# NVlabs/motion-policy-networks

Measured on AMD Instinct MI355X. Metric: env-steps/sec (FK+SDF+PointNet++), higher is better.
Workload: dtype f32

## Files before the change

### motion-policy-networks_amd/csrc/sa3_chain.hip

```cpp
#include "common.h"

#include <type_traits>

typedef float f32x16 __attribute__((ext_vector_type(16)));
typedef unsigned int u32x4 __attribute__((ext_vector_type(4)));

namespace sa3 {
constexpr int ROWS = 128, PR = 64, WV = 4;

template <int K1, int C1, int C2, int C3>
struct Cfg {
  static_assert(K1 % 8 == 0 && K1 % 16 == 0, "input rows are whole 16-float slabs");
  static_assert(C1 == 128 * WV && C2 == 128 * WV && C3 == 256 * WV, "a wave owns 128 channels (256 of the last layer)");
  static constexpr int KG1 = K1 / 8, KG2 = C1 / 8, KG3 = C2 / 8;
  static constexpr int64_t W1_OFF = 0, W2_OFF = (int64_t)C1 * K1, W3_OFF = W2_OFF + (int64_t)C2 * C1;
  static constexpr int64_t B1_OFF = W3_OFF + (int64_t)C3 * C2, B2_OFF = B1_OFF + C1, B3_OFF = B2_OFF + C2;
  static constexpr int64_t TOTAL = B3_OFF + C3;
  static constexpr int KMAX = K1 > C1 ? (K1 > C2 ? K1 : C2) : (C1 > C2 ? C1 : C2);
  static constexpr int LD = KMAX + 4;
  static constexpr int LDS_BYTES = PR * LD * 4;
};
}

template <class C>
__global__ void __launch_bounds__(256)
    sa3_pack_kernel(const float *__restrict__ w1, int k1_real, const float *__restrict__ b1, const float *__restrict__ w2,
                    const float *__restrict__ b2, const float *__restrict__ w3, const float *__restrict__ b3, int K1, int C1,
                    int C2, int C3, float *__restrict__ pack) {
  const int64_t e = (int64_t)blockIdx.x * 256 + threadIdx.x;
  if (e >= C::TOTAL) return;
  float v;
  if (e >= C::B1_OFF) {
    const int64_t i = e - C::B1_OFF;
    v = i < C1 ? b1[i] : (i < C1 + C2 ? b2[i - C1] : b3[i - C1 - C2]);
  } else {
    const float *w;
    int kin, kreal, KG;
    int64_t r = e;
    if (r >= C::W3_OFF) { r -= C::W3_OFF; w = w3; kin = C2; kreal = C2; KG = C::KG3; }
    else if (r >= C::W2_OFF) { r -= C::W2_OFF; w = w2; kin = C1; kreal = C1; KG = C::KG2; }
    else { w = w1; kin = K1; kreal = k1_real; KG = C::KG1; }
    const int i = (int)(r & 3), lane = (int)((r >> 2) & 63), ot = (int)((r >> 8) & 3);
    const int64_t ug = r >> 10;
    const int g = (int)(ug % KG), unit = (int)(ug / KG);
    const int out = unit * 128 + ot * 32 + (lane & 31), in = 8 * g + 4 * (lane >> 5) + i;
    (void)kin;
    v = in < kreal ? w[(size_t)out * kreal + in] : 0.0f;
  }
  pack[e] = v;
}

__device__ __forceinline__ f32x16 sa3_mfma(float a, float b, f32x16 c) { return __builtin_amdgcn_mfma_f32_32x32x2f32(a, b, c, 0, 0, 0); }
__device__ __forceinline__ float4 sa3_bload16(__amdgpu_buffer_rsrc_t rsrc, int voff, int soff) {
  const u32x4 r = __builtin_amdgcn_raw_buffer_load_b128(rsrc, voff, soff, 0);
  return make_float4(__uint_as_float(r.x), __uint_as_float(r.y), __uint_as_float(r.z), __uint_as_float(r.w));
}
template <int I, int E, class F>
__device__ __forceinline__ void static_for(F &&f) {
  if constexpr (I < E) {
    f(std::integral_constant<int, I>{});
    static_for<I + 1, E>(f);
  }
}
__device__ __forceinline__ float sa3_comp(const float4 &q, int i) { return i == 0 ? q.x : (i == 1 ? q.y : (i == 2 ? q.z : q.w)); }

template <int K1, int C1, int C2, int C3, bool PROBE = false>
__global__ void __launch_bounds__(64 * sa3::WV) __attribute__((amdgpu_waves_per_eu(1, 1)))
    sa3_chain_kernel(const float *__restrict__ x, int ldx, const float *__restrict__ pack, float *__restrict__ out, int ldo,
                     long long *__restrict__ probe = nullptr) {
  using C = sa3::Cfg<K1, C1, C2, C3>;
  using namespace sa3;
  extern __shared__ __attribute__((aligned(16))) float H[];
  constexpr int LD = C::LD;
  const int tid = threadIdx.x, lane = tid & 63;
  const int wave = __builtin_amdgcn_readfirstlane(tid >> 6);
  const int half = lane >> 5, col = lane & 31;
  const int64_t env = blockIdx.x;
  const __amdgpu_buffer_rsrc_t rsrc =
      __builtin_amdgcn_make_buffer_rsrc(const_cast<float *>(pack), 0, (int)(C::TOTAL * 4), 0x00020000);
  const int voff = lane * 16;
  const float *hrow0 = H + col * LD + 4 * half;
  float pool[2][4];
#pragma unroll
  for (int hf = 0; hf < 2; ++hf)
#pragma unroll
    for (int ot = 0; ot < 4; ++ot) pool[hf][ot] = -__builtin_inff();

  auto run = [&](auto KGt, auto FLIPt, int wbase, f32x16 (&acc)[4][2]) __attribute__((always_inline)) {
    constexpr int KG = decltype(KGt)::value;
    constexpr bool FLIP = decltype(FLIPt)::value;
    constexpr int NS = 4;
    float4 wr[NS][4], br[NS][2];
    auto fetch = [&](int st, int g) __attribute__((always_inline)) {
      const int soff = wbase + g * 4096;
#pragma unroll
      for (int ot = 0; ot < 4; ++ot) wr[st][ot] = sa3_bload16(rsrc, voff + ot * 1024, soff);
      br[st][0] = *reinterpret_cast<const float4 *>(hrow0 + 8 * g);
      br[st][1] = *reinterpret_cast<const float4 *>(hrow0 + 32 * LD + 8 * g);
    };
    auto compute = [&](int st) __attribute__((always_inline)) {
#pragma unroll
      for (int i = 0; i < 4; ++i)
#pragma unroll
        for (int ot = 0; ot < 4; ++ot)
#pragma unroll
          for (int rt = 0; rt < 2; ++rt) {
            const float w = sa3_comp(wr[st][ot], i), a = sa3_comp(br[st][rt], i);
            acc[ot][rt] = FLIP ? sa3_mfma(w, a, acc[ot][rt]) : sa3_mfma(a, w, acc[ot][rt]);
          }
    };
#pragma unroll
    for (int st = 0; st < NS - 1; ++st) fetch(st, st);
    auto issue_order = [&]() __attribute__((always_inline)) {
#pragma unroll
      for (int k = 0; k < 4; ++k) {
        __builtin_amdgcn_sched_group_barrier(0x008, 4, 0);
        __builtin_amdgcn_sched_group_barrier(0x020, 1, 0);
      }
#pragma unroll
      for (int k = 0; k < 2; ++k) {
        __builtin_amdgcn_sched_group_barrier(0x008, 4, 0);
        __builtin_amdgcn_sched_group_barrier(0x100, 1, 0);
      }
      __builtin_amdgcn_sched_group_barrier(0x008, 8, 0);
    };
    constexpr int ROUNDS = (KG - NS + 1) / NS;
    for (int r = 0; r < ROUNDS; ++r) {
#pragma unroll
      for (int st = 0; st < NS; ++st) {
        fetch((st + NS - 1) % NS, r * NS + st + NS - 1);
        compute(st);
        issue_order();
      }
    }
    static_for<ROUNDS * NS, KG>([&](auto G) __attribute__((always_inline)) {
      constexpr int g = decltype(G)::value;
      if constexpr (g + NS - 1 < KG) {
        fetch((g + NS - 1) % NS, g + NS - 1);
        compute(g % NS);
        issue_order();
      } else {
        compute(g % NS);
      }
    });
  };
  auto bias_init = [&](int boff_floats, f32x16 (&acc)[4][2]) __attribute__((always_inline)) {
#pragma unroll
    for (int ot = 0; ot < 4; ++ot)
#pragma unroll
      for (int j = 0; j < 4; ++j) {
        const float4 b = sa3_bload16(rsrc, half * 16, (boff_floats + wave * 128 + ot * 32 + 8 * j) * 4);
#pragma unroll
        for (int rt = 0; rt < 2; ++rt) {
          acc[ot][rt][4 * j + 0] = b.x, acc[ot][rt][4 * j + 1] = b.y, acc[ot][rt][4 * j + 2] = b.z, acc[ot][rt][4 * j + 3] = b.w;
        }
      }
  };
  auto write_back = [&](const f32x16 (&acc)[4][2]) __attribute__((always_inline)) {
#pragma unroll
    for (int rt = 0; rt < 2; ++rt)
#pragma unroll
      for (int ot = 0; ot < 4; ++ot)
#pragma unroll
        for (int j = 0; j < 4; ++j) {
          float4 v;
          v.x = fmaxf(acc[ot][rt][4 * j + 0], 0.0f), v.y = fmaxf(acc[ot][rt][4 * j + 1], 0.0f);
          v.z = fmaxf(acc[ot][rt][4 * j + 2], 0.0f), v.w = fmaxf(acc[ot][rt][4 * j + 3], 0.0f);
          *reinterpret_cast<float4 *>(H + (rt * 32 + col) * LD + wave * 128 + ot * 32 + 8 * j + 4 * half) = v;
        }
  };

  int pi = 0;
  auto stamp = [&]() __attribute__((always_inline)) {
    if constexpr (PROBE) {
      if (blockIdx.x == 300 && tid == 0) probe[pi] = (long long)__builtin_amdgcn_s_memtime();
      ++pi;
    }
  };
  stamp();
  for (int pass = 0; pass < ROWS / PR; ++pass) {
    const float *xr = x + (env * ROWS + pass * PR) * (int64_t)ldx;
    constexpr int NX = PR * (K1 / 4) / (64 * WV);
    static_assert(NX * 64 * WV == PR * (K1 / 4), "the input rows split evenly over the threads");
    {
      float4 xb[NX];
#pragma unroll
      for (int j = 0; j < NX; ++j) {
        const int i = tid + j * 64 * WV, r = i / (K1 / 4), c4 = i - r * (K1 / 4);
        xb[j] = *reinterpret_cast<const float4 *>(xr + (int64_t)r * ldx + 4 * c4);
      }
#pragma unroll
      for (int j = 0; j < NX; ++j) {
        const int i = tid + j * 64 * WV, r = i / (K1 / 4), c4 = i - r * (K1 / 4);
        *reinterpret_cast<float4 *>(H + r * LD + 4 * c4) = xb[j];
      }
    }
    __syncthreads();
    stamp();
    f32x16 acc[4][2];
    bias_init((int)C::B1_OFF, acc);
    run(std::integral_constant<int, C::KG1>{}, std::true_type{}, (int)(C::W1_OFF * 4) + wave * C::KG1 * 4096, acc);
    stamp();
    __syncthreads();
    write_back(acc);
    __syncthreads();
    stamp();
    bias_init((int)C::B2_OFF, acc);
    run(std::integral_constant<int, C::KG2>{}, std::true_type{}, (int)(C::W2_OFF * 4) + wave * C::KG2 * 4096, acc);
    stamp();
    __syncthreads();
    write_back(acc);
    __syncthreads();
    stamp();
#pragma unroll
    for (int hf = 0; hf < 2; ++hf) {
#pragma unroll
      for (int ot = 0; ot < 4; ++ot)
#pragma unroll
        for (int rt = 0; rt < 2; ++rt) acc[ot][rt] = f32x16{0, 0, 0, 0, 0, 0, 0, 0, 0, 0, 0, 0, 0, 0, 0, 0};
      run(std::integral_constant<int, C::KG3>{}, std::false_type{}, (int)(C::W3_OFF * 4) + (wave * 2 + hf) * C::KG3 * 4096, acc);
#pragma unroll
      for (int ot = 0; ot < 4; ++ot) {
        float m = fmaxf(acc[ot][0][0], acc[ot][1][0]);
#pragma unroll
        for (int r = 1; r < 16; ++r) m = fmaxf(m, fmaxf(acc[ot][0][r], acc[ot][1][r]));
        pool[hf][ot] = fmaxf(pool[hf][ot], m);
      }
      stamp();
    }
    __syncthreads();
    stamp();
  }
  const float *b3 = pack + C::B3_OFF;
#pragma unroll
  for (int hf = 0; hf < 2; ++hf)
#pragma unroll
    for (int ot = 0; ot < 4; ++ot) {
      const float v = mpx_max_across_halves(pool[hf][ot]);
      const int ch = wave * 256 + hf * 128 + ot * 32 + col;
      if (half == 0) out[env * (int64_t)ldo + ch] = fmaxf(v + b3[ch], 0.0f);
    }
}

#define SA3_DISPATCH(CALL)                                                                              \
  if (K1 == 272 && c1 == 512 && c2 == 512 && c3 == 1024) { CALL(272, 512, 512, 1024); }                 \
  else {                                                                                                \
    mpx_set_error("mpx_sa3: unsupported group-all MLP (K1=%d, %d, %d, %d)", K1, c1, c2, c3);            \
    return 1;                                                                                           \
  }

MPX_EXPORT int64_t mpx_sa3_pack_size(int K1, int c1, int c2, int c3) {
  if (K1 == 272 && c1 == 512 && c2 == 512 && c3 == 1024) return sa3::Cfg<272, 512, 512, 1024>::TOTAL;
  return -1;
}

MPX_EXPORT int mpx_sa3_pack_weights(const float *w1, int k1_real, const float *b1, const float *w2, const float *b2,
                                    const float *w3, const float *b3, int K1, int c1, int c2, int c3, float *pack,
                                    mpx_stream_t stream) {
  MPX_REQUIRE(w1 && b1 && w2 && b2 && w3 && b3 && pack, "mpx_sa3_pack_weights: NULL operand");
  MPX_REQUIRE(k1_real >= 1 && k1_real <= K1, "mpx_sa3_pack_weights: the real input width %d must be in [1, K1 = %d]", k1_real, K1);
#define CALL(a, b, c, d)                                                                                             \
  do {                                                                                                               \
    using C = sa3::Cfg<a, b, c, d>;                                                                                  \
    hipLaunchKernelGGL(sa3_pack_kernel<C>, dim3(cdiv(C::TOTAL, 256)), dim3(256), 0, mpx_s(stream), w1, k1_real, b1, w2, \
                       b2, w3, b3, K1, c1, c2, c3, pack);                                                            \
    MPX_LAUNCH_CHECK("mpx_sa3_pack_weights");                                                                        \
  } while (0)
  SA3_DISPATCH(CALL)
#undef CALL
}

MPX_EXPORT int mpx_sa3_chain_probe(const float *x, int ldx, int B, const float *pack, float *out, int ldo, int64_t *probe,
                                   mpx_stream_t stream) {
  using C = sa3::Cfg<272, 512, 512, 1024>;
  MPX_LDS_LIMIT_ONCE((sa3_chain_kernel<272, 512, 512, 1024, true>), C::LDS_BYTES, "mpx_sa3_chain_probe");
  hipLaunchKernelGGL((sa3_chain_kernel<272, 512, 512, 1024, true>), dim3((unsigned)B), dim3(64 * sa3::WV), C::LDS_BYTES,
                     mpx_s(stream), x, ldx, pack, out, ldo, reinterpret_cast<long long *>(probe));
  MPX_LAUNCH_CHECK("mpx_sa3_chain_probe");
}

MPX_EXPORT int mpx_sa3_chain(const float *x, int ldx, int B, int rows, const float *pack, int K1, int c1, int c2, int c3,
                             float *out, int ldo, mpx_stream_t stream) {
  MPX_REQUIRE(B >= 0 && x && pack && out, "mpx_sa3_chain: bad operand");
  MPX_REQUIRE(rows == sa3::ROWS, "mpx_sa3_chain: the module pools exactly %d rows per environment (got %d)", sa3::ROWS, rows);
  MPX_REQUIRE(ldx >= K1 && ldx % 4 == 0 && ldo >= c3, "mpx_sa3_chain: bad leading dimension");
  MPX_REQUIRE((((uintptr_t)x | (uintptr_t)pack) & 15) == 0, "mpx_sa3_chain: x and pack must be 16-byte aligned");
  if (B == 0) return 0;
#define CALL(a, b, c, d)                                                                                            \
  do {                                                                                                              \
    using C = sa3::Cfg<a, b, c, d>;                                                                                 \
    MPX_LDS_LIMIT_ONCE((sa3_chain_kernel<a, b, c, d>), C::LDS_BYTES, "mpx_sa3_chain");                              \
    hipLaunchKernelGGL((sa3_chain_kernel<a, b, c, d>), dim3((unsigned)B), dim3(64 * sa3::WV), C::LDS_BYTES,        \
                       mpx_s(stream), x, ldx, pack, out, ldo, (long long *)nullptr);                                \
    MPX_LAUNCH_CHECK("mpx_sa3_chain");                                                                              \
  } while (0)
  SA3_DISPATCH(CALL)
#undef CALL
}
```

### motion-policy-networks_amd/csrc/launch_routes.h

```cpp
#pragma once
#include <stdint.h>

static inline int cdiv(int64_t a, int64_t b) { return (int)((a + b - 1) / b); }

#ifndef MPX_FPS4_MIN_B
#define MPX_FPS4_MIN_B 768
#endif
constexpr int FPS_MAX_N = 8192;
constexpr int FPS_MAX_LDS = 256 + 3 * FPS_MAX_N * 4;
constexpr int FPSC_CELLS = 4096;
constexpr int64_t fpsc_lds_bytes(int N, bool nocloud = false) {
  const int64_t cloud = nocloud ? 0 : (int64_t)3 * N * 4, pro = (int64_t)FPSC_CELLS * 4 + (((int64_t)N * 2 + 15) & ~(int64_t)15);
  return 768 + (cloud > pro ? cloud : pro);
}
inline int opt_n_threads_log2(int n) {
  int l = 0;
  while ((2 << l) <= n && (2 << l) <= 512) ++l;
  return l;
}

enum { FPS_PLAIN = 0, FPS_WAVE = 1, FPS_CULL8 = 2, FPS_CULL4 = 3 };
struct FpsRoute {
  int family;
  int pts;
  int threads;
  int lds;
};
inline FpsRoute fps_route(int B, int N, int fast) {
  if (fast && N <= 512) {
    switch ((N + 63) / 64) {
      case 1: return {FPS_WAVE, 1, 64, 0};
      case 2: return {FPS_WAVE, 2, 64, 0};
      case 3: case 4: return {FPS_WAVE, 4, 64, 0};
      default: return {FPS_WAVE, 8, 64, 0};
    }
  }
  if (fast && N > 512) {
    const int waves = (N > 16 * 256 && B >= MPX_FPS4_MIN_B) ? 4 : 8;
    const int lds_c = (int)fpsc_lds_bytes(N, waves == 4);
    const int pts_c = (N + 64 * waves - 1) / (64 * waves);
    if (waves == 4) return {FPS_CULL4, pts_c <= 20 ? 20 : pts_c <= 25 ? 25 : 32, 256, lds_c};
    const int p = pts_c <= 2 ? 2 : pts_c <= 4 ? 4 : pts_c <= 6 ? 6 : pts_c <= 8 ? 8 : pts_c <= 10 ? 10 : pts_c <= 13 ? 13 : 16;
    return {FPS_CULL8, p, 512, lds_c};
  }
  int block = ((N + 63) / 64) * 64;
  if (block > 512) block = 512;
  const int pts = (N + block - 1) / block;
  const int lds = 256 + 3 * N * 4;
  switch (pts) {
    case 1: case 2: case 3: case 4: case 5: case 6: case 7: case 8: return {FPS_PLAIN, pts, block, lds};
    case 9: case 10: return {FPS_PLAIN, 10, block, lds};
    case 11: case 12: case 13: return {FPS_PLAIN, 13, block, lds};
    case 14: case 15: case 16: return {FPS_PLAIN, 16, block, lds};
    default: return {FPS_PLAIN, 0, block, lds};
  }
}

constexpr int COL_PPB = 16;
#ifndef MPX_COL_TC
#define MPX_COL_TC 64
#endif
static_assert(MPX_COL_TC >= 1 && MPX_COL_TC <= 64 && MPX_COL_TC * 64 <= 16 * 256,
              "MPX_COL_TC: FK runs on one thread per waypoint of a chunk and a thread holds at most 16 (waypoint, sphere) pairs");

enum { COL_NONE = 0, COL_GENERAL = 1, COL_WAVE = 2, COL_ENV = 3 };
struct CollisionRoute {
  int form;
  int ppt;
  int block;
  int tc;
  int chunks;
  int last;
};
inline CollisionRoute collision_route(int B, int T, int S, int M1, int M2, bool frames_aligned) {
  if (B == 0 || T == 0 || S == 0) return {COL_NONE, 0, 0, 0, 0, 0};
  if (M1 <= 64 && M2 <= 64 && S <= 64 && frames_aligned) {
    const bool wave = T * S <= 64;
    const int tc = wave ? 64 : MPX_COL_TC;
    const int chunks = cdiv(T, tc), last = (T - (chunks - 1) * tc) * S;
    if (wave) return {COL_WAVE, 1, 64, tc, chunks, last};
    const int sel = ((T < tc ? T : tc) * S + 511) / 512;
    return {COL_ENV, sel >= 1 && sel <= 7 ? 2 * sel : 16, 256, tc, chunks, last};
  }
  const int groups = cdiv((int64_t)B * T, COL_PPB);
  return {COL_GENERAL, 0, 256, 0, groups, (int)((int64_t)B * T - (int64_t)(groups - 1) * COL_PPB) * S};
}

constexpr int LINEAR_BM = 128, LINEAR_BN = 128;
inline bool gemv_fits(int M, int K) { return M <= 8 && (int64_t)(M <= 1 ? 1 : M <= 2 ? 2 : M <= 4 ? 4 : 8) * K * 4 <= 64 * 1024; }
// ... 101 lines not shown
```

### motion-policy-networks_amd/csrc/pointnet.hip

```cpp
#include "common.h"

#include <stdlib.h>
#include <type_traits>

typedef unsigned long long u64;

template <int CTRL>
__device__ __forceinline__ u64 dpp_mov64(u64 v) {
  unsigned lo = (unsigned)v, hi = (unsigned)(v >> 32);
  lo = (unsigned)__builtin_amdgcn_update_dpp(0, (int)lo, CTRL, 0xf, 0xf, true);
  hi = (unsigned)__builtin_amdgcn_update_dpp(0, (int)hi, CTRL, 0xf, 0xf, true);
  return ((u64)hi << 32) | lo;
}
struct U32Pair {
  unsigned lo, hi;
};
__device__ __forceinline__ u64 pack64(unsigned lo, unsigned hi) { return __builtin_bit_cast(u64, U32Pair{lo, hi}); }
__device__ __forceinline__ u64 umax64(u64 a, u64 b) {
  double r;
  asm("v_max_f64 %0, %1, %2" : "=v"(r) : "v"(__builtin_bit_cast(double, a)), "v"(__builtin_bit_cast(double, b)));
  return __builtin_bit_cast(u64, r);
}

__device__ __forceinline__ u64 row_max64(u64 v) {
  v = umax64(v, dpp_mov64<0xB1>(v));
  v = umax64(v, dpp_mov64<0x4E>(v));
  v = umax64(v, dpp_mov64<0x141>(v));
  v = umax64(v, dpp_mov64<0x140>(v));
  return v;
}
__device__ __forceinline__ u64 readlane64(u64 v, int lane) {
  unsigned lo = (unsigned)__builtin_amdgcn_readlane((int)(unsigned)v, lane);
  unsigned hi = (unsigned)__builtin_amdgcn_readlane((int)(unsigned)(v >> 32), lane);
  return ((u64)hi << 32) | lo;
}
__device__ __forceinline__ u64 wave_max64(u64 v) {
  v = row_max64(v);
  u64 a = umax64(readlane64(v, 0), readlane64(v, 16));
  u64 b = umax64(readlane64(v, 32), readlane64(v, 48));
  return umax64(a, b);
}

template <int PTS>
__global__ void __launch_bounds__(1024) __attribute__((amdgpu_waves_per_eu(PTS <= 8 ? 8 : 4, PTS <= 8 ? 8 : 4)))
    fps_kernel(const float *__restrict__ xyz, int N, int stride, int npoint, int log2bs,
               int32_t *__restrict__ idx, float *__restrict__ new_xyz, int new_stride) {
  extern __shared__ __attribute__((aligned(16))) unsigned char smem[];
  u64 *slots = reinterpret_cast<u64 *>(smem);
  float *sx = reinterpret_cast<float *>(smem + 256);
  float *sy = sx + N;
  float *sz = sy + N;

  const int b = blockIdx.x;
  const int tid = threadIdx.x;
  const int nthr = blockDim.x;
  const int lane = tid & 63;
  const int wave = tid >> 6;
  const float *pts = xyz + (size_t)b * N * stride;
  int32_t *out = idx + (size_t)b * npoint;
  float *nxyz = new_xyz ? new_xyz + (size_t)b * npoint * new_stride : nullptr;
  const unsigned bsmask = (1u << log2bs) - 1u;

  float x[PTS], y[PTS], z[PTS];
  u64 key[PTS];
#pragma unroll
  for (int i = 0; i < PTS; ++i) {
    const int k = tid + i * nthr;
    x[i] = y[i] = z[i] = 0.0f;
    key[i] = 0;
    if (k < N) {
      x[i] = pts[(size_t)k * stride + 0];
      y[i] = pts[(size_t)k * stride + 1];
      z[i] = pts[(size_t)k * stride + 2];
      sx[k] = x[i];
      sy[k] = y[i];
      sz[k] = z[i];
      const float mag = mpx_sqdist(x[i], y[i], z[i]);
      if (!((double)mag <= 1e-3)) {
        const unsigned rank = (__brev((unsigned)k & bsmask) & 0xFFFF0000u) | ((unsigned)k >> log2bs);
        key[i] = pack64(0xFFFFFFFFu - rank, __float_as_uint(1e10f));
      }
    }
  }
  if (tid < 32) slots[tid] = 0;
  __syncthreads();

  int old = 0;
  for (int j = 1; j < npoint; ++j) {
    const float x1 = sx[old], y1 = sy[old], z1 = sz[old];
    if (tid == 0) {
      out[j - 1] = old;
      if (nxyz) {
        nxyz[(size_t)(j - 1) * new_stride + 0] = x1;
        nxyz[(size_t)(j - 1) * new_stride + 1] = y1;
        nxyz[(size_t)(j - 1) * new_stride + 2] = z1;
      }
    }
    u64 best = 0;
#pragma unroll
    for (int i = 0; i < PTS; ++i) {
      const float dx = x[i] - x1, dy = y[i] - y1, dz = z[i] - z1;
      const float d = mpx_sqdist(dx, dy, dz);
      float d2;
// ... 73 lines not shown
      if (nxyz) {
        nxyz[(size_t)(j - 1) * new_stride + 0] = x1;
        nxyz[(size_t)(j - 1) * new_stride + 1] = y1;
        nxyz[(size_t)(j - 1) * new_stride + 2] = z1;
      }
    }
    u64 best = 0;
#pragma unroll
    for (int i = 0; i < PTS; ++i) {
      const float dx = x[i] - x1, dy = y[i] - y1, dz = z[i] - z1;
      const float d = mpx_sqdist(dx, dy, dz);
      float d2;
      asm("v_min_f32 %0, %1, %2" : "=v"(d2) : "v"(d), "v"(__uint_as_float((unsigned)(key[i] >> 32))));
      key[i] = pack64((unsigned)key[i], __float_as_uint(d2));
      best = umax64(best, key[i]);
    }
    const u64 m = wave_max64(best);
    if (m == 0) {
      old = 0;
    } else {
      const unsigned rank = 0xFFFFFFFFu - (unsigned)m;
      old = (int)(((rank & 0xFFFFu) << log2bs) | __brev(rank & 0xFFFF0000u));
    }
  }
  if (npoint > 0) {
    float x1, y1, z1;
    coords(old, x1, y1, z1);
    if (lane == 0) {
      out[npoint - 1] = old;
      if (nxyz) {
        nxyz[(size_t)(npoint - 1) * new_stride + 0] = x1;
        nxyz[(size_t)(npoint - 1) * new_stride + 1] = y1;
        nxyz[(size_t)(npoint - 1) * new_stride + 2] = z1;
      }
    }
  }
}

template <int CTRL>
__device__ __forceinline__ float dpp_movf(float v) {
  return __uint_as_float((unsigned)__builtin_amdgcn_update_dpp(0, (int)__float_as_uint(v), CTRL, 0xf, 0xf, true));
}
template <bool MAX>
__device__ __forceinline__ float wave_red_f32(float v) {
  auto op = [](float a, float b) { return MAX ? fmaxf(a, b) : fminf(a, b); };
  v = op(v, dpp_movf<0xB1>(v));
  v = op(v, dpp_movf<0x4E>(v));
  v = op(v, dpp_movf<0x141>(v));
  v = op(v, dpp_movf<0x140>(v));
  auto rl = [&](int l) { return __uint_as_float((unsigned)__builtin_amdgcn_readlane((int)__float_as_uint(v), l)); };
  return op(op(rl(0), rl(16)), op(rl(32), rl(48)));
}
__device__ __forceinline__ unsigned writelane_u32(unsigned s, int lane, unsigned v) {
  const unsigned su = (unsigned)__builtin_amdgcn_readfirstlane((int)s);
#define MPX_WL(L) case L: asm("v_writelane_b32 %0, %1, " #L : "+v"(v) : "s"(su)); break;
  switch (lane) {
    MPX_WL(0) MPX_WL(1) MPX_WL(2) MPX_WL(3) MPX_WL(4) MPX_WL(5) MPX_WL(6) MPX_WL(7)
    MPX_WL(8) MPX_WL(9) MPX_WL(10) MPX_WL(11) MPX_WL(12) MPX_WL(13) MPX_WL(14) MPX_WL(15)
    MPX_WL(16) MPX_WL(17) MPX_WL(18) MPX_WL(19) MPX_WL(20) MPX_WL(21) MPX_WL(22) MPX_WL(23)
    MPX_WL(24) MPX_WL(25) MPX_WL(26) MPX_WL(27) MPX_WL(28) MPX_WL(29) MPX_WL(30) MPX_WL(31)
    default: break;
  }
#undef MPX_WL
  return v;
}
__device__ __forceinline__ float writelane_f32(float s, int lane, float v) {
  return __uint_as_float(writelane_u32(__float_as_uint(s), lane, __float_as_uint(v)));
}
__device__ __forceinline__ u64 writelane64(u64 s, int lane, u64 v) {
  return pack64(writelane_u32((unsigned)s, lane, (unsigned)v), writelane_u32((unsigned)(s >> 32), lane, (unsigned)(v >> 32)));
}
__device__ __forceinline__ unsigned morton4(unsigned v) {
  v &= 0xFu;
  v = (v | (v << 4)) & 0xC3u;
  v = (v | (v << 2)) & 0x249u;
  return v;
}

template <int I, int E, class F>
__device__ __forceinline__ void static_for(F &&f) {
  if constexpr (I < E) {
    f(std::integral_constant<int, I>{});
    static_for<I + 1, E>(f);
  }
}

__device__ __forceinline__ unsigned wave_max_u32_dpp(unsigned v) {
  asm volatile(
      "s_nop 1\n\tv_max_u32_dpp %0, %0, %0 quad_perm:[1,0,3,2] row_mask:0xf bank_mask:0xf\n\t"
      "s_nop 1\n\tv_max_u32_dpp %0, %0, %0 quad_perm:[2,3,0,1] row_mask:0xf bank_mask:0xf\n\t"
      "s_nop 1\n\tv_max_u32_dpp %0, %0, %0 row_half_mirror row_mask:0xf bank_mask:0xf\n\t"
      "s_nop 1\n\tv_max_u32_dpp %0, %0, %0 row_mirror row_mask:0xf bank_mask:0xf\n\t"
      "s_nop 1\n\tv_max_u32_dpp %0, %0, %0 row_bcast:15 row_mask:0xa bank_mask:0xf\n\t"
      "s_nop 1\n\tv_max_u32_dpp %0, %0, %0 row_bcast:31 row_mask:0xc bank_mask:0xf\n\t"
      "s_nop 1"
      : "+v"(v));
  return (unsigned)__builtin_amdgcn_readlane((int)v, 63);
}
__device__ __forceinline__ u64 wave_max64_staged(u64 k) {
  const unsigned hi = (unsigned)(k >> 32), lo = (unsigned)k;
  const unsigned mhi = wave_max_u32_dpp(hi);
  const unsigned mlo = wave_max_u32_dpp(hi == mhi ? lo : 0u);
  return pack64(mlo, mhi);
}

template <int PTS, int FPSC_WAVES>
__global__ void __launch_bounds__(64 * FPSC_WAVES)
    __attribute__((amdgpu_waves_per_eu(FPSC_WAVES == 4 ? 3 : FPSC_WAVES / 2, FPSC_WAVES == 4 ? 3 : FPSC_WAVES / 2)))
    fps_cull_kernel(const float *__restrict__ xyz, int N, int stride, int npoint, int32_t *__restrict__ idx,
                    float *__restrict__ new_xyz, int new_stride) {
  static_assert(PTS >= 2 && PTS <= 32, "slots per lane");
  static_assert(FPSC_WAVES == 4 || FPSC_WAVES == 8 || FPSC_WAVES == 16, "4 x 25, 8 x 13 or 16 x 7 points per lane");
  constexpr int FPSC_THREADS = 64 * FPSC_WAVES, CPT = FPSC_CELLS / FPSC_THREADS;
  constexpr bool NOCLOUD = FPSC_WAVES == 4;
  extern __shared__ __attribute__((aligned(16))) unsigned char smem[];
  u64 *slots = reinterpret_cast<u64 *>(smem);
  int *scal = reinterpret_cast<int *>(smem + 256);
  float *bbx = reinterpret_cast<float *>(smem + 256 + 16);
  unsigned *hist = reinterpret_cast<unsigned *>(smem + 768);
  unsigned short *pmap = reinterpret_cast<unsigned short *>(smem + 768 + FPSC_CELLS * 4);
  float *sx = reinterpret_cast<float *>(smem + 768), *sy = sx + N, *sz = sy + N;

  const int b = blockIdx.x, tid = threadIdx.x, lane = tid & 63;
  const int wave = __builtin_amdgcn_readfirstlane(tid >> 6);
  const float *pts = xyz + (size_t)b * N * stride;
  int32_t *out = idx + (size_t)b * npoint;
  float *nxyz = new_xyz ? new_xyz + (size_t)b * npoint * new_stride : nullptr;
  const float INF = __builtin_inff();

  unsigned code[PTS], rnk[PTS];
  {
    float x[PTS], y[PTS], z[PTS];
    float mn[3] = {INF, INF, INF}, mx[3] = {-INF, -INF, -INF};
#pragma unroll
    for (int i = 0; i < PTS; ++i) {
      const int k = tid + i * FPSC_THREADS;
      x[i] = y[i] = z[i] = 0.0f;
      if (k < N) {
        x[i] = pts[(size_t)k * stride + 0];
        y[i] = pts[(size_t)k * stride + 1];
        z[i] = pts[(size_t)k * stride + 2];
        mn[0] = fminf(mn[0], x[i]), mn[1] = fminf(mn[1], y[i]), mn[2] = fminf(mn[2], z[i]);
        mx[0] = fmaxf(mx[0], x[i]), mx[1] = fmaxf(mx[1], y[i]), mx[2] = fmaxf(mx[2], z[i]);
      }
    }
#pragma unroll
    for (int c = 0; c < 3; ++c) {
      mn[c] = wave_red_f32<false>(mn[c]);
      mx[c] = wave_red_f32<true>(mx[c]);
    }
    if (lane == 0) {
#pragma unroll
      for (int c = 0; c < 3; ++c) bbx[wave * 6 + c] = mn[c], bbx[wave * 6 + 3 + c] = mx[c];
    }
    for (int i = tid; i < FPSC_CELLS; i += FPSC_THREADS) hist[i] = 0;
    if (tid < 32) slots[tid] = 0;
    __syncthreads();
#pragma unroll
    for (int w = 0; w < FPSC_WAVES; ++w)
#pragma unroll
      for (int c = 0; c < 3; ++c) mn[c] = fminf(mn[c], bbx[w * 6 + c]), mx[c] = fmaxf(mx[c], bbx[w * 6 + 3 + c]);
    float sc[3];
#pragma unroll
    for (int c = 0; c < 3; ++c) sc[c] = mx[c] > mn[c] ? 16.0f * __builtin_amdgcn_rcpf(mx[c] - mn[c]) : 0.0f;
#pragma unroll
    for (int i = 0; i < PTS; ++i) {
// ... 33 lines not shown
    for (int e = 0; e < CPT; ++e) {
      hist[tid * CPT + e] = base;
      base += c8[e];
    }
    __syncthreads();
  }
#pragma unroll
  for (int i = 0; i < PTS; ++i) {
    const int k = tid + i * FPSC_THREADS;
    if (k < N) {
      const unsigned pos = hist[code[i]] + rnk[i];
      pmap[pos] = (unsigned short)k;
      if (k == 0) scal[0] = (int)pos;
    }
  }
  __syncthreads();

  float x[PTS], y[PTS], z[PTS];
  u64 key[PTS];
  int kk[PTS];
  static_for<0, PTS>([&](auto I) {
    constexpr int i = decltype(I)::value;
    const int pos = (wave + FPSC_WAVES * i) * 64 + lane;
    kk[i] = pos < N ? (int)pmap[pos] : -1;
  });
  const int pos0 = scal[0];
  __syncthreads();
  static_for<0, PTS>([&](auto I) {
    constexpr int i = decltype(I)::value;
    const int pos = (wave + FPSC_WAVES * i) * 64 + lane;
    x[i] = y[i] = z[i] = 0.0f;
    key[i] = 0;
    if (kk[i] >= 0) {
      const int k = kk[i];
      x[i] = pts[(size_t)k * stride + 0];
      y[i] = pts[(size_t)k * stride + 1];
      z[i] = pts[(size_t)k * stride + 2];
      if constexpr (!NOCLOUD) {
        sx[pos] = x[i];
        sy[pos] = y[i];
        sz[pos] = z[i];
      }
      const float mag = mpx_sqdist(x[i], y[i], z[i]);
      if (!((double)mag <= 1e-3)) {
        const unsigned rank = (__brev((unsigned)k & 511u) & 0xFF800000u) | (((unsigned)k >> 9) << 18) | (unsigned)pos;
        key[i] = pack64(0xFFFFFFFFu - rank, __float_as_uint(1e10f));
      }
    }
  });
  float bnx = INF, bny = INF, bnz = INF, bxx = -INF, bxy = -INF, bxz = -INF, cub = 0.0f;
  __syncthreads();
  if constexpr (NOCLOUD) {
    static_for<0, PTS>([&](auto I) {
      constexpr int i = decltype(I)::value;
      const bool real = (wave + FPSC_WAVES * i) * 64 + lane < N;
      const float mnx_ = wave_red_f32<false>(real ? x[i] : INF), mny_ = wave_red_f32<false>(real ? y[i] : INF),
                  mnz_ = wave_red_f32<false>(real ? z[i] : INF), mxx_ = wave_red_f32<true>(real ? x[i] : -INF),
                  mxy_ = wave_red_f32<true>(real ? y[i] : -INF), mxz_ = wave_red_f32<true>(real ? z[i] : -INF);
      const bool any = __builtin_amdgcn_ballot_w64(key[i] != 0) != 0;
      if (lane == i) {
        bnx = mnx_, bny = mny_, bnz = mnz_, bxx = mxx_, bxy = mxy_, bxz = mxz_;
        cub = any ? 1e10f : 0.0f;
      }
    });
  } else if (lane < PTS) {
    const int p0 = (wave + FPSC_WAVES * lane) * 64;
    if (p0 < N) {
      bool any = false;
#pragma unroll 8
      for (int q = 0; q < 64; ++q) {
        const int pos = min(p0 + ((q + 5 * lane) & 63), N - 1);
        const float px = sx[pos], py = sy[pos], pz = sz[pos];
        bnx = fminf(bnx, px), bny = fminf(bny, py), bnz = fminf(bnz, pz);
        bxx = fmaxf(bxx, px), bxy = fmaxf(bxy, py), bxz = fmaxf(bxz, pz);
        const float mag = mpx_sqdist(px, py, pz);
        any = any || !((double)mag <= 1e-3);
      }
      cub = any ? 1e10f : 0.0f;
    }
  }

  int old = 0, pos_old = pos0;
  float cx1 = pts[0], cy1 = pts[1], cz1 = pts[2];
  for (int j = 1; j < npoint; ++j) {
    float x1, y1, z1;
    if constexpr (NOCLOUD) {
      x1 = cx1, y1 = cy1, z1 = cz1;
    } else {
      x1 = sx[pos_old], y1 = sy[pos_old], z1 = sz[pos_old];
    }
    if (tid == 0) {
      out[j - 1] = old;
      if (nxyz) {
        nxyz[(size_t)(j - 1) * new_stride + 0] = x1;
        nxyz[(size_t)(j - 1) * new_stride + 1] = y1;
        nxyz[(size_t)(j - 1) * new_stride + 2] = z1;
      }
    }
    const float ax = bnx - x1, bx_ = x1 - bxx, ay = bny - y1, by_ = y1 - bxy, az = bnz - z1, bz_ = z1 - bxz;
    const float ex = fmaxf(fmaxf(ax, bx_), 0.0f), ey = fmaxf(fmaxf(ay, by_), 0.0f), ez = fmaxf(fmaxf(az, bz_), 0.0f);
    const float bound = mpx_sqdist(ex, ey, ez);
    const unsigned tmask = (unsigned)__builtin_amdgcn_ballot_w64(lane < PTS && bound < cub);
    {
      const float fx = fmaxf(-ax, -bx_), fy = fmaxf(-ay, -by_), fz = fmaxf(-az, -bz_);
      const float far = mpx_sqdist(fx, fy, fz) * 1.000001f;
      cub = fminf(cub, far);
    }
    static_for<0, PTS>([&](auto I) {
      constexpr int i = decltype(I)::value;
      if (tmask & (1u << i)) {
        const float dx = x[i] - x1, dy = y[i] - y1, dz = z[i] - z1;
        const float d = mpx_sqdist(dx, dy, dz);
        float d2;
        asm("v_min_f32 %0, %1, %2" : "=v"(d2) : "v"(d), "v"(__uint_as_float((unsigned)(key[i] >> 32))));
        key[i] = pack64((unsigned)key[i], __float_as_uint(d2));
      }
    });
    u64 best;
    {
      u64 b0 = key[0], b1 = key[1];
      static_for<1, (PTS + 1) / 2>([&](auto I) {
        constexpr int i = 2 * decltype(I)::value;
        b0 = umax64(b0, key[i]);
        if constexpr (i + 1 < PTS) b1 = umax64(b1, key[i + 1]);
      });
      best = umax64(b0, b1);
    }
    best = wave_max64_staged(best);
    u64 *slot = slots + (j & 1) * 16;
    if (lane == 0) slot[wave] = best;
    __syncthreads();
    u64 m = row_max64(slot[lane & 15]);
    m = readlane64(m, 0);
    if (m == 0) {
      old = 0;
      pos_old = pos0;
    } else {
      const unsigned rank = 0xFFFFFFFFu - (unsigned)m;
      old = (int)((((rank >> 18) & 0x1Fu) << 9) | __brev(rank & 0xFF800000u));
      pos_old = (int)(rank & 0x1FFFu);
    }
    if constexpr (NOCLOUD) {
      const float *pp = pts + (size_t)old * stride;
      cx1 = pp[0], cy1 = pp[1], cz1 = pp[2];
    }
  }
  if (tid == 0 && npoint > 0) {
    out[npoint - 1] = old;
    if (nxyz) {
      nxyz[(size_t)(npoint - 1) * new_stride + 0] = NOCLOUD ? cx1 : sx[pos_old];
      nxyz[(size_t)(npoint - 1) * new_stride + 1] = NOCLOUD ? cy1 : sy[pos_old];
      nxyz[(size_t)(npoint - 1) * new_stride + 2] = NOCLOUD ? cz1 : sz[pos_old];
    }
  }
}

static std::atomic<int> g_variant[MPX_VARIANT_COUNT_] = {{1}, {1}, {1}, {1}};
MPX_EXPORT int mpx_set_variant(int what, int value) {
  MPX_REQUIRE(what >= 0 && what < MPX_VARIANT_COUNT_, "mpx_set_variant: unknown selector %d", what);
  MPX_REQUIRE(value == 0 || value == 1, "mpx_set_variant: value must be 0 (plain kernels) or 1 (default)");
  g_variant[what].store(value, std::memory_order_relaxed);
  if (what == MPX_VARIANT_UNIT_QUEUE) mpx_unit_queue_set_slots(value ? 256 : 0);
  return 0;
}
MPX_EXPORT int mpx_get_variant(int what) {
  return (what >= 0 && what < MPX_VARIANT_COUNT_) ? g_variant[what].load(std::memory_order_relaxed) : -1;
// ... 629 lines not shown
```

Before: 99020.

## Make SA3 chain kernel persistent and prefetch next layer's weights and inputs

The SA3 MLP chain kernel becomes persistent: it launches one workgroup per CU and loops over environments instead of one block per environment. The weight pipeline prologue and bias loads for the next layer are issued before the barriers and LDS write-back. The next pass's input rows are fetched with buffer loads in the middle of the last layer's GEMM, hiding global latency across layers and environments. This adds register pressure from the hoisted prefetch buffers and relies on the CU count for load balance, with possible tail imbalance when B is not a multiple of the CU count.

```diff
diff --git a/motion-policy-networks_amd/csrc/sa3_chain.hip b/motion-policy-networks_amd/csrc/sa3_chain.hip
--- a/motion-policy-networks_amd/csrc/sa3_chain.hip
+++ b/motion-policy-networks_amd/csrc/sa3_chain.hip
@@ -66,8 +66,8 @@
 
 template <int K1, int C1, int C2, int C3, bool PROBE = false>
 __global__ void __launch_bounds__(64 * sa3::WV) __attribute__((amdgpu_waves_per_eu(1, 1)))
-    sa3_chain_kernel(const float *__restrict__ x, int ldx, const float *__restrict__ pack, float *__restrict__ out, int ldo,
-                     long long *__restrict__ probe = nullptr) {
+    sa3_chain_kernel(const float *__restrict__ x, int ldx, int B, const float *__restrict__ pack, float *__restrict__ out,
+                     int ldo, long long *__restrict__ probe = nullptr) {
   using C = sa3::Cfg<K1, C1, C2, C3>;
   using namespace sa3;
   extern __shared__ __attribute__((aligned(16))) float H[];
@@ -75,29 +75,61 @@
   const int tid = threadIdx.x, lane = tid & 63;
   const int wave = __builtin_amdgcn_readfirstlane(tid >> 6);
   const int half = lane >> 5, col = lane & 31;
-  const int64_t env = blockIdx.x;
   const __amdgpu_buffer_rsrc_t rsrc =
       __builtin_amdgcn_make_buffer_rsrc(const_cast<float *>(pack), 0, (int)(C::TOTAL * 4), 0x00020000);
   const int voff = lane * 16;
   const float *hrow0 = H + col * LD + 4 * half;
+  constexpr int NS = 4;
+  float4 wr[NS][4], br[NS][2];
+  float4 bq[4][4];
+  constexpr int NX = PR * (K1 / 4) / (64 * WV);
+  static_assert(NX * 64 * WV == PR * (K1 / 4), "the input rows split evenly over the threads");
+  u32x4 xb[NX];
   float pool[2][4];
-#pragma unroll
-  for (int hf = 0; hf < 2; ++hf)
-#pragma unroll
-    for (int ot = 0; ot < 4; ++ot) pool[hf][ot] = -__builtin_inff();
-
-  auto run = [&](auto KGt, auto FLIPt, int wbase, f32x16 (&acc)[4][2]) __attribute__((always_inline)) {
+
+  auto fetch_w = [&](int st, int wbase, int g) __attribute__((always_inline)) {
+    const int soff = wbase + g * 4096;
+#pragma unroll
+    for (int ot = 0; ot < 4; ++ot) wr[st][ot] = sa3_bload16(rsrc, voff + ot * 1024, soff);
+  };
+  auto fetch_l = [&](int st, int g) __attribute__((always_inline)) {
+    br[st][0] = *reinterpret_cast<const float4 *>(hrow0 + 8 * g);
+    br[st][1] = *reinterpret_cast<const float4 *>(hrow0 + 32 * LD + 8 * g);
+  };
+  auto preload_w = [&](int wbase) __attribute__((always_inline)) {
+#pragma unroll
+    for (int st = 0; st < NS - 1; ++st) fetch_w(st, wbase, st);
+  };
+  auto bias_load = [&](int boff_floats) __attribute__((always_inline)) {
+#pragma unroll
+    for (int ot = 0; ot < 4; ++ot)
+#pragma unroll
+      for (int j = 0; j < 4; ++j) bq[ot][j] = sa3_bload16(rsrc, half * 16, (boff_floats + wave * 128 + ot * 32 + 8 * j) * 4);
+  };
+  auto bias_apply = [&](f32x16 (&acc)[4][2]) __attribute__((always_inline)) {
+#pragma unroll
+    for (int ot = 0; ot < 4; ++ot)
+#pragma unroll
+      for (int j = 0; j < 4; ++j)
+#pragma unroll
+        for (int rt = 0; rt < 2; ++rt) {
+          acc[ot][rt][4 * j + 0] = bq[ot][j].x, acc[ot][rt][4 * j + 1] = bq[ot][j].y;
+          acc[ot][rt][4 * j + 2] = bq[ot][j].z, acc[ot][rt][4 * j + 3] = bq[ot][j].w;
+        }
+  };
+#define SA3_LOAD_X(ENV, PASS)                                                                                        \
+  do {                                                                                                               \
+    const __amdgpu_buffer_rsrc_t xrs_ = __builtin_amdgcn_make_buffer_rsrc(                                           \
+        const_cast<float *>(x + ((ENV) * ROWS + (PASS) * PR) * (int64_t)ldx), 0, ((PR - 1) * ldx + K1) * 4, 0x00020000); \
+    _Pragma("unroll") for (int j = 0; j < NX; ++j) {                                                                 \
+      const int i = tid + j * 64 * WV, r = i / (K1 / 4), c4 = i - r * (K1 / 4);                                      \
+      xb[j] = __builtin_amdgcn_raw_buffer_load_b128(xrs_, (r * ldx + 4 * c4) * 4, 0, 0);                             \
+    }                                                                                                                \
+  } while (0)
+  auto run = [&](auto KGt, auto FLIPt, auto PARTt, int wbase, f32x16 (&acc)[4][2]) __attribute__((always_inline)) {
+    constexpr int PART = decltype(PARTt)::value;
     constexpr int KG = decltype(KGt)::value;
     constexpr bool FLIP = decltype(FLIPt)::value;
-    constexpr int NS = 4;
-    float4 wr[NS][4], br[NS][2];
-    auto fetch = [&](int st, int g) __attribute__((always_inline)) {
-      const int soff = wbase + g * 4096;
-#pragma unroll
-      for (int ot = 0; ot < 4; ++ot) wr[st][ot] = sa3_bload16(rsrc, voff + ot * 1024, soff);
-      br[st][0] = *reinterpret_cast<const float4 *>(hrow0 + 8 * g);
-      br[st][1] = *reinterpret_cast<const float4 *>(hrow0 + 32 * LD + 8 * g);
-    };
     auto compute = [&](int st) __attribute__((always_inline)) {
 #pragma unroll
       for (int i = 0; i < 4; ++i)
@@ -109,8 +141,10 @@
             acc[ot][rt] = FLIP ? sa3_mfma(w, a, acc[ot][rt]) : sa3_mfma(a, w, acc[ot][rt]);
           }
     };
-#pragma unroll
-    for (int st = 0; st < NS - 1; ++st) fetch(st, st);
+    if constexpr (PART != 2) {
+#pragma unroll
+      for (int st = 0; st < NS - 1; ++st) fetch_l(st, st);
+    }
     auto issue_order = [&]() __attribute__((always_inline)) {
 #pragma unroll
       for (int k = 0; k < 4; ++k) {
@@ -125,36 +159,28 @@
       __builtin_amdgcn_sched_group_barrier(0x008, 8, 0);
     };
     constexpr int ROUNDS = (KG - NS + 1) / NS;
-    for (int r = 0; r < ROUNDS; ++r) {
+    constexpr int RB = PART == 2 ? ROUNDS / 2 : 0, RE = PART == 1 ? ROUNDS / 2 : ROUNDS;
+    auto round = [&](int r) __attribute__((always_inline)) {
 #pragma unroll
       for (int st = 0; st < NS; ++st) {
-        fetch((st + NS - 1) % NS, r * NS + st + NS - 1);
+        fetch_w((st + NS - 1) % NS, wbase, r * NS + st + NS - 1);
+        fetch_l((st + NS - 1) % NS, r * NS + st + NS - 1);
         compute(st);
         issue_order();
       }
-    }
-    static_for<ROUNDS * NS, KG>([&](auto G) __attribute__((always_inline)) {
+    };
+    for (int r = RB; r < RE; ++r) round(r);
+    static_for<(PART == 1 ? KG : ROUNDS * NS), KG>([&](auto G) __attribute__((always_inline)) {
       constexpr int g = decltype(G)::value;
       if constexpr (g + NS - 1 < KG) {
-        fetch((g + NS - 1) % NS, g + NS - 1);
+        fetch_w((g + NS - 1) % NS, wbase, g + NS - 1);
+        fetch_l((g + NS - 1) % NS, g + NS - 1);
         compute(g % NS);
         issue_order();
       } else {
         compute(g % NS);
       }
     });
-  };
-  auto bias_init = [&](int boff_floats, f32x16 (&acc)[4][2]) __attribute__((always_inline)) {
-#pragma unroll
-    for (int ot = 0; ot < 4; ++ot)
-#pragma unroll
-      for (int j = 0; j < 4; ++j) {
-        const float4 b = sa3_bload16(rsrc, half * 16, (boff_floats + wave * 128 + ot * 32 + 8 * j) * 4);
-#pragma unroll
-        for (int rt = 0; rt < 2; ++rt) {
-          acc[ot][rt][4 * j + 0] = b.x, acc[ot][rt][4 * j + 1] = b.y, acc[ot][rt][4 * j + 2] = b.z, acc[ot][rt][4 * j + 3] = b.w;
-        }
-      }
   };
   auto write_back = [&](const f32x16 (&acc)[4][2]) __attribute__((always_inline)) {
 #pragma unroll
@@ -169,80 +195,104 @@
           *reinterpret_cast<float4 *>(H + (rt * 32 + col) * LD + wave * 128 + ot * 32 + 8 * j + 4 * half) = v;
         }
   };
+  using P0 = std::integral_constant<int, 0>;
+  const int w1 = (int)(C::W1_OFF * 4) + wave * C::KG1 * 4096, w2 = (int)(C::W2_OFF * 4) + wave * C::KG2 * 4096;
+  const int w3 = (int)(C::W3_OFF * 4) + wave * 2 * C::KG3 * 4096;
+  const float *b3 = pack + C::B3_OFF;
 
   int pi = 0;
+  bool probe_on = false;
   auto stamp = [&]() __attribute__((always_inline)) {
     if constexpr (PROBE) {
-      if (blockIdx.x == 300 && tid == 0) probe[pi] = (long long)__builtin_amdgcn_s_memtime();
+      __builtin_amdgcn_sched_barrier(0);
+      probe[probe_on ? pi : 31] = (long long)__builtin_amdgcn_s_memtime();
+      __builtin_amdgcn_sched_barrier(0);
       ++pi;
     }
   };
-  stamp();
-  for (int pass = 0; pass < ROWS / PR; ++pass) {
-    const float *xr = x + (env * ROWS + pass * PR) * (int64_t)ldx;
-    constexpr int NX = PR * (K1 / 4) / (64 * WV);
-    static_assert(NX * 64 * WV == PR * (K1 / 4), "the input rows split evenly over the threads");
-    {
-      float4 xb[NX];
+  const int grid = gridDim.x;
+  bias_load((int)C::B1_OFF);
+  preload_w(w1);
+  SA3_LOAD_X((int64_t)blockIdx.x, 0);
+  for (int64_t env = blockIdx.x; env < B; env += grid) {
+    if constexpr (PROBE) {
+      probe_on = wave == 0 && (int)blockIdx.x == grid / 2 && env == (int64_t)blockIdx.x + grid;
+      pi = 0;
+    }
+    stamp();
+#pragma unroll
+    for (int hf = 0; hf < 2; ++hf)
+#pragma unroll
+      for (int ot = 0; ot < 4; ++ot) pool[hf][ot] = -__builtin_inff();
+    for (int pass = 0; pass < ROWS / PR; ++pass) {
 #pragma unroll
       for (int j = 0; j < NX; ++j) {
         const int i = tid + j * 64 * WV, r = i / (K1 / 4), c4 = i - r * (K1 / 4);
-        xb[j] = *reinterpret_cast<const float4 *>(xr + (int64_t)r * ldx + 4 * c4);
-      }
-#pragma unroll
-      for (int j = 0; j < NX; ++j) {
-        const int i = tid + j * 64 * WV, r = i / (K1 / 4), c4 = i - r * (K1 / 4);
-        *reinterpret_cast<float4 *>(H + r * LD + 4 * c4) = xb[j];
-      }
+        *reinterpret_cast<u32x4 *>(H + r * LD + 4 * c4) = xb[j];
+      }
+      __syncthreads();
+      stamp();
+      f32x16 acc[4][2];
+      bias_apply(acc);
+      run(std::integral_constant<int, C::KG1>{}, std::true_type{}, P0{}, w1, acc);
+      stamp();
+      bias_load((int)C::B2_OFF);
+      preload_w(w2);
+      __syncthreads();
+      write_back(acc);
+      __syncthreads();
+      stamp();
+      bias_apply(acc);
+      run(std::integral_constant<int, C::KG2>{}, std::true_type{}, P0{}, w2, acc);
+      stamp();
+      preload_w(w3);
+      __syncthreads();
+      write_back(acc);
+      __syncthreads();
+      stamp();
+      const int64_t nenv = pass + 1 < ROWS / PR ? env : env + grid;
+      const int npass = pass + 1 < ROWS / PR ? pass + 1 : 0;
+#pragma unroll
+      for (int hf = 0; hf < 2; ++hf) {
+#pragma unroll
+        for (int ot = 0; ot < 4; ++ot)
+#pragma unroll
+          for (int rt = 0; rt < 2; ++rt) acc[ot][rt] = f32x16{0, 0, 0, 0, 0, 0, 0, 0, 0, 0, 0, 0, 0, 0, 0, 0};
+        if (hf == 0) {
+          run(std::integral_constant<int, C::KG3>{}, std::false_type{}, P0{}, w3, acc);
+          preload_w(w3 + C::KG3 * 4096);
+        } else {
+          run(std::integral_constant<int, C::KG3>{}, std::false_type{}, std::integral_constant<int, 1>{}, w3 + C::KG3 * 4096, acc);
+          if (nenv < B) SA3_LOAD_X(nenv, npass);
+          run(std::integral_constant<int, C::KG3>{}, std::false_type{}, std::integral_constant<int, 2>{}, w3 + C::KG3 * 4096, acc);
+          bias_load((int)C::B1_OFF);
+          preload_w(w1);
+        }
+#pragma unroll
+        for (int ot = 0; ot < 4; ++ot) {
+          float m = fmaxf(acc[ot][0][0], acc[ot][1][0]);
+#pragma unroll
+          for (int r = 1; r < 16; ++r) m = fmaxf(m, fmaxf(acc[ot][0][r], acc[ot][1][r]));
+          pool[hf][ot] = fmaxf(pool[hf][ot], m);
+        }
+        stamp();
+      }
+      __syncthreads();
+      stamp();
     }
-    __syncthreads();
-    stamp();
-    f32x16 acc[4][2];
-    bias_init((int)C::B1_OFF, acc);
-    run(std::integral_constant<int, C::KG1>{}, std::true_type{}, (int)(C::W1_OFF * 4) + wave * C::KG1 * 4096, acc);
-    stamp();
-    __syncthreads();
-    write_back(acc);
-    __syncthreads();
-    stamp();
-    bias_init((int)C::B2_OFF, acc);
-    run(std::integral_constant<int, C::KG2>{}, std::true_type{}, (int)(C::W2_OFF * 4) + wave * C::KG2 * 4096, acc);
-    stamp();
-    __syncthreads();
-    write_back(acc);
-    __syncthreads();
-    stamp();
-#pragma unroll
-    for (int hf = 0; hf < 2; ++hf) {
-#pragma unroll
-      for (int ot = 0; ot < 4; ++ot)
-#pragma unroll
-        for (int rt = 0; rt < 2; ++rt) acc[ot][rt] = f32x16{0, 0, 0, 0, 0, 0, 0, 0, 0, 0, 0, 0, 0, 0, 0, 0};
-      run(std::integral_constant<int, C::KG3>{}, std::false_type{}, (int)(C::W3_OFF * 4) + (wave * 2 + hf) * C::KG3 * 4096, acc);
+#pragma unroll
+    for (int hf = 0; hf < 2; ++hf)
 #pragma unroll
       for (int ot = 0; ot < 4; ++ot) {
-        float m = fmaxf(acc[ot][0][0], acc[ot][1][0]);
-#pragma unroll
-        for (int r = 1; r < 16; ++r) m = fmaxf(m, fmaxf(acc[ot][0][r], acc[ot][1][r]));
-        pool[hf][ot] = fmaxf(pool[hf][ot], m);
-      }
-      stamp();
-    }
-    __syncthreads();
-    stamp();
+        const float v = mpx_max_across_halves(pool[hf][ot]);
+        const int ch = wave * 256 + hf * 128 + ot * 32 + col;
+        if (half == 0) out[env * (int64_t)ldo + ch] = fmaxf(v + b3[ch], 0.0f);
+      }
   }
-  const float *b3 = pack + C::B3_OFF;
-#pragma unroll
-  for (int hf = 0; hf < 2; ++hf)
-#pragma unroll
-    for (int ot = 0; ot < 4; ++ot) {
-      const float v = mpx_max_across_halves(pool[hf][ot]);
-      const int ch = wave * 256 + hf * 128 + ot * 32 + col;
-      if (half == 0) out[env * (int64_t)ldo + ch] = fmaxf(v + b3[ch], 0.0f);
-    }
-}
-
-#define SA3_DISPATCH(CALL)                                                                              \
+#undef SA3_LOAD_X
+}
+
+#define SA3_DISPATCH(CALL)                                                                             \
   if (K1 == 272 && c1 == 512 && c2 == 512 && c3 == 1024) { CALL(272, 512, 512, 1024); }                 \
   else {                                                                                                \
     mpx_set_error("mpx_sa3: unsupported group-all MLP (K1=%d, %d, %d, %d)", K1, c1, c2, c3);            \
@@ -273,9 +323,12 @@
 MPX_EXPORT int mpx_sa3_chain_probe(const float *x, int ldx, int B, const float *pack, float *out, int ldo, int64_t *probe,
                                    mpx_stream_t stream) {
   using C = sa3::Cfg<272, 512, 512, 1024>;
+  const int cus = mpx_cu_count();
+  MPX_REQUIRE(cus > 0, "mpx_sa3_chain_probe: the device does not report its compute units");
+  MPX_REQUIRE(B >= 2 * cus, "mpx_sa3_chain_probe: the probe stamps a workgroup's second environment (B >= %d)", 2 * cus);
   MPX_LDS_LIMIT_ONCE((sa3_chain_kernel<272, 512, 512, 1024, true>), C::LDS_BYTES, "mpx_sa3_chain_probe");
-  hipLaunchKernelGGL((sa3_chain_kernel<272, 512, 512, 1024, true>), dim3((unsigned)B), dim3(64 * sa3::WV), C::LDS_BYTES,
-                     mpx_s(stream), x, ldx, pack, out, ldo, reinterpret_cast<long long *>(probe));
+  hipLaunchKernelGGL((sa3_chain_kernel<272, 512, 512, 1024, true>), dim3((unsigned)cus), dim3(64 * sa3::WV), C::LDS_BYTES,
+                     mpx_s(stream), x, ldx, B, pack, out, ldo, reinterpret_cast<long long *>(probe));
   MPX_LAUNCH_CHECK("mpx_sa3_chain_probe");
 }
 
@@ -283,15 +336,18 @@
                              float *out, int ldo, mpx_stream_t stream) {
   MPX_REQUIRE(B >= 0 && x && pack && out, "mpx_sa3_chain: bad operand");
   MPX_REQUIRE(rows == sa3::ROWS, "mpx_sa3_chain: the module pools exactly %d rows per environment (got %d)", sa3::ROWS, rows);
-  MPX_REQUIRE(ldx >= K1 && ldx % 4 == 0 && ldo >= c3, "mpx_sa3_chain: bad leading dimension");
+  MPX_REQUIRE(ldx >= K1 && ldx % 4 == 0 && ldx <= (1 << 22) && ldo >= c3, "mpx_sa3_chain: bad leading dimension");
   MPX_REQUIRE((((uintptr_t)x | (uintptr_t)pack) & 15) == 0, "mpx_sa3_chain: x and pack must be 16-byte aligned");
   if (B == 0) return 0;
+  const int cus = mpx_cu_count();
+  MPX_REQUIRE(cus > 0, "mpx_sa3_chain: the device does not report its compute units");
+  const int grid = B < cus ? B : cus;
 #define CALL(a, b, c, d)                                                                                            \
   do {                                                                                                              \
     using C = sa3::Cfg<a, b, c, d>;                                                                                 \
-    MPX_LDS_LIMIT_ONCE((sa3_chain_kernel<a, b, c, d>), C::LDS_BYTES, "mpx_sa3_chain");                              \
-    hipLaunchKernelGGL((sa3_chain_kernel<a, b, c, d>), dim3((unsigned)B), dim3(64 * sa3::WV), C::LDS_BYTES,        \
-                       mpx_s(stream), x, ldx, pack, out, ldo, (long long *)nullptr);                                \
+    MPX_LDS_LIMIT_ONCE((sa3_chain_kernel<a, b, c, d>), C::LDS_BYTES, "mpx_sa3_chain");                           \
+    hipLaunchKernelGGL((sa3_chain_kernel<a, b, c, d>), dim3((unsigned)grid), dim3(64 * sa3::WV), C::LDS_BYTES,  \
+                       mpx_s(stream), x, ldx, B, pack, out, ldo, (long long *)nullptr);                             \
     MPX_LAUNCH_CHECK("mpx_sa3_chain");                                                                              \
   } while (0)
   SA3_DISPATCH(CALL)
```

Result: no change. 99730 (median of 6 runs) (+0.7%).

## Select two farthest points per FPS round in the 4-wave culled kernel

Applied to the files above, without the earlier changes.

Adds a paired-selection path to the NOCLOUD 4-wave culled farthest-point-sampling kernel. Each round it tracks the top two keys per lane and per wave, then accepts the runner-up as the next sample when its distance to the new winner does not lower its key. When that holds, two FPS iterations are committed per block-wide reduction and barrier. In exchange, every update computes two distances per point and reduces two maxima, and the acceptance test must exactly reproduce sequential FPS ordering.

```diff
diff --git a/motion-policy-networks_amd/csrc/launch_routes.h b/motion-policy-networks_amd/csrc/launch_routes.h
--- a/motion-policy-networks_amd/csrc/launch_routes.h
+++ b/motion-policy-networks_amd/csrc/launch_routes.h
@@ -5,6 +5,9 @@
 
 #ifndef MPX_FPS4_MIN_B
 #define MPX_FPS4_MIN_B 768
+#endif
+#ifndef MPX_FPS4_PAIR
+#define MPX_FPS4_PAIR 1
 #endif
 constexpr int FPS_MAX_N = 8192;
 constexpr int FPS_MAX_LDS = 256 + 3 * FPS_MAX_N * 4;
diff --git a/motion-policy-networks_amd/csrc/pointnet.hip b/motion-policy-networks_amd/csrc/pointnet.hip
--- a/motion-policy-networks_amd/csrc/pointnet.hip
+++ b/motion-policy-networks_amd/csrc/pointnet.hip
@@ -19,6 +19,11 @@
 __device__ __forceinline__ u64 umax64(u64 a, u64 b) {
   double r;
   asm("v_max_f64 %0, %1, %2" : "=v"(r) : "v"(__builtin_bit_cast(double, a)), "v"(__builtin_bit_cast(double, b)));
+  return __builtin_bit_cast(u64, r);
+}
+__device__ __forceinline__ u64 umin64(u64 a, u64 b) {
+  double r;
+  asm("v_min_f64 %0, %1, %2" : "=v"(r) : "v"(__builtin_bit_cast(double, a)), "v"(__builtin_bit_cast(double, b)));
   return __builtin_bit_cast(u64, r);
 }
 
@@ -258,6 +263,14 @@
   if constexpr (I < E) {
     f(std::integral_constant<int, I>{});
     static_for<I + 1, E>(f);
+  }
+}
+
+template <int I, int E>
+__device__ __forceinline__ void pin_slots(float (&x)[E], float (&y)[E], float (&z)[E], u64 (&key)[E]) {
+  if constexpr (I < E) {
+    asm volatile("" : "+v"(x[I]), "+v"(y[I]), "+v"(z[I]), "+v"(key[I]));
+    pin_slots<I + 1>(x, y, z, key);
   }
 }
 
@@ -457,6 +470,109 @@
 
   int old = 0, pos_old = pos0;
   float cx1 = pts[0], cy1 = pts[1], cz1 = pts[2];
+  if constexpr (NOCLOUD) {
+    pin_slots<0>(x, y, z, key);
+    asm volatile("" : "+v"(bnx), "+v"(bny), "+v"(bnz), "+v"(bxx), "+v"(bxy), "+v"(bxz), "+v"(cub));
+  }
+  if constexpr (NOCLOUD && MPX_FPS4_PAIR != 0) {
+    int cnt = 1, old2 = 0;
+    bool two = false;
+    float cx2 = cx1, cy2 = cy1, cz2 = cz1;
+    auto box = [&](float px, float py, float pz, float &bound, float &far) {
+      const float ax = bnx - px, bx_ = px - bxx, ay = bny - py, by_ = py - bxy, az = bnz - pz, bz_ = pz - bxz;
+      const float ex = fmaxf(fmaxf(ax, bx_), 0.0f), ey = fmaxf(fmaxf(ay, by_), 0.0f), ez = fmaxf(fmaxf(az, bz_), 0.0f);
+      bound = mpx_sqdist(ex, ey, ez);
+      const float fx = fmaxf(-ax, -bx_), fy = fmaxf(-ay, -by_), fz = fmaxf(-az, -bz_);
+      far = mpx_sqdist(fx, fy, fz) * 1.000001f;
+    };
+    auto put = [&](int j, int k, float px, float py, float pz) {
+      out[j] = k;
+      if (nxyz) {
+        nxyz[(size_t)j * new_stride + 0] = px;
+        nxyz[(size_t)j * new_stride + 1] = py;
+        nxyz[(size_t)j * new_stride + 2] = pz;
+      }
+    };
+    auto decode = [](u64 m) {
+      const unsigned rank = 0xFFFFFFFFu - (unsigned)m;
+      return (int)((((rank >> 18) & 0x1Fu) << 9) | __brev(rank & 0xFF800000u));
+    };
+    for (unsigned rnd = 0; cnt < npoint; ++rnd) {
+      if (tid == 0) {
+        put(cnt - (two ? 2 : 1), old, cx1, cy1, cz1);
+        if (two) put(cnt - 1, old2, cx2, cy2, cz2);
+      }
+      float bound, far;
+      box(cx1, cy1, cz1, bound, far);
+      bool hit = bound < cub;
+      if (two) {
+        float bound2, far2;
+        box(cx2, cy2, cz2, bound2, far2);
+        hit = hit || bound2 < cub;
+        far = fminf(far, far2);
+      }
+      const unsigned tmask = (unsigned)__builtin_amdgcn_ballot_w64(lane < PTS && hit);
+      cub = fminf(cub, far);
+      static_for<0, PTS>([&](auto I) {
+        constexpr int i = decltype(I)::value;
+        if (tmask & (1u << i)) {
+          const float da = mpx_sqdist(x[i] - cx1, y[i] - cy1, z[i] - cz1), db = mpx_sqdist(x[i] - cx2, y[i] - cy2, z[i] - cz2);
+          float d2;
+          asm("v_min_f32 %0, %1, %2" : "=v"(d2) : "v"(da), "v"(__uint_as_float((unsigned)(key[i] >> 32))));
+          asm("v_min_f32 %0, %1, %2" : "=v"(d2) : "v"(db), "v"(d2));
+          key[i] = pack64((unsigned)key[i], __float_as_uint(d2));
+        }
+      });
+      u64 m1, m2;
+      if constexpr (MPX_FPS4_PAIR == 2) {
+        u64 e1 = key[0], e2 = 0, o1 = key[1], o2 = 0;
+        static_for<1, (PTS + 1) / 2>([&](auto I) {
+          constexpr int i = 2 * decltype(I)::value;
+          e2 = umax64(e2, umin64(e1, key[i]));
+          e1 = umax64(e1, key[i]);
+          if constexpr (i + 1 < PTS) {
+            o2 = umax64(o2, umin64(o1, key[i + 1]));
+            o1 = umax64(o1, key[i + 1]);
+          }
+        });
+        m1 = umax64(e1, o1);
+        m2 = umax64(umin64(e1, o1), umax64(e2, o2));
+      } else {
+        m1 = umax64(key[0], key[1]), m2 = umin64(key[0], key[1]);
+        static_for<2, PTS>([&](auto I) {
+          constexpr int i = decltype(I)::value;
+          m2 = umax64(m2, umin64(m1, key[i]));
+          m1 = umax64(m1, key[i]);
+        });
+      }
+      const u64 w1 = wave_max64_staged(m1);
+      const u64 w2 = wave_max64_staged(m1 == w1 ? m2 : m1);
+      u64 *slot = slots + (rnd & 1) * 16;
+      if (lane == 0) slot[2 * wave] = w1, slot[2 * wave + 1] = w2;
+      __syncthreads();
+      const u64 e = slot[lane & 15];
+      const u64 ma = readlane64(row_max64(e), 0);
+      const u64 mb = readlane64(row_max64(e == ma ? 0 : e), 0);
+      old = ma == 0 ? 0 : decode(ma);
+      const int nb = mb == 0 ? 0 : decode(mb);
+      const float *pa = pts + (size_t)old * stride, *pb = pts + (size_t)nb * stride;
+      cx1 = pa[0], cy1 = pa[1], cz1 = pa[2];
+      const float bx = pb[0], by = pb[1], bz = pb[2];
+      ++cnt;
+      const unsigned dist_b = (unsigned)(mb >> 32);
+      float keep;
+      asm("v_min_f32 %0, %1, %2" : "=v"(keep) : "v"(mpx_sqdist(bx - cx1, by - cy1, bz - cz1)), "v"(__uint_as_float(dist_b)));
+      two = cnt < npoint && mb > (ma & 0xFFFFFFFFull) &&
+            (unsigned)__builtin_amdgcn_readfirstlane((int)__float_as_uint(keep)) == dist_b;
+      old2 = two ? nb : old, cx2 = two ? bx : cx1, cy2 = two ? by : cy1, cz2 = two ? bz : cz1;
+      cnt += two ? 1 : 0;
+    }
+    if (tid == 0 && npoint > 0) {
+      put(cnt - (two ? 2 : 1), old, cx1, cy1, cz1);
+      if (two) put(cnt - 1, old2, cx2, cy2, cz2);
+    }
+    return;
+  }
   for (int j = 1; j < npoint; ++j) {
     float x1, y1, z1;
     if constexpr (NOCLOUD) {
```

Measured after the change: 99060 before, 99360 after, median of 6. Within noise of the previous version (+0.3%).
